# cbg-ethz/LongSom

Hardware: AMD Instinct MI355X
Metric: genomic sites/s pileup+call, 10M-read BAM x 5k barcodes, 1/2/4/8 MI355X (higher is better)
Workload: dtype u32

## Files before the change

### longsom_amd/csrc/pileup.hip

```cpp
#include "lsg_ctx.h"
#include <hipcub/hipcub.hpp>
#include <cstdio>
#include <cstdlib>
#include <cstring>

namespace lsg {

#define LSG_AS3 __attribute__((address_space(3)))
__device__ __forceinline__ uint32_t lds_addr(const void* p) { return (uint32_t)(uintptr_t)(LSG_AS3 const void*)p; }
constexpr int ARENA = 256;

enum { SC_COLS = 8, SC_OVERFLOW = 9, SC_READS = 10, SC_SEGS = 11, SC_EVENTS = 12, SC_ROWS_DEEP = 15,
       SC_ROWS = 16, SC_ROWS_SRC = 28, SC_NENT = 38, SC_QWALK = 48,
       SC_ROWALLOC = 160, SC_ROWALLOC_STRIDE = 16, SC_COUNT = SC_ROWALLOC + SC_ROWALLOC_STRIDE * LSG_MAX_CELLTYPES };

struct CountArgs {
    int64_t n_reads;
    const int32_t* read_tid; const uint16_t* read_flag; const uint8_t* read_mapq; const int32_t* read_cb;
    const int64_t* contig_len; const uint8_t* const* ref_ptr;
    const uint8_t* celltype_of;
    int32_t n_contigs, n_cb, n_ct;
    uint32_t tile_lo, tile_hi;
    int32_t min_bq, min_mq, min_dp, min_cc, ignore_orphans;
    uint32_t flag_exclude;
// ... 15 lines not shown
    unsigned long long n_ok = 0;
    for (int64_t r = (int64_t)blockIdx.x * blockDim.x + threadIdx.x; r < a.n_reads; r += (int64_t)gridDim.x * blockDim.x) {
        const uint32_t flag = a.read_flag[r];
        const int32_t cb = a.read_cb[r], tid = a.read_tid[r];
        bool pass = (flag & a.flag_exclude) == 0 && (int)a.read_mapq[r] >= a.min_mq;
        if (pass && a.ignore_orphans && (flag & 0x1) && !(flag & 0x2)) pass = false;
        if (pass && a.read_drop && a.read_drop[r] == 1) pass = false;
        if (a.adm) {
            const unsigned long long m = __ballot(pass);
            if ((threadIdx.x & 63) == 0) a.adm[r >> 6] = m;
        }
        bool ok = pass && cb >= 0 && cb < a.n_cb && tid >= 0 && tid < a.n_contigs;
        if (ok && a.celltype_of[cb] >= (uint32_t)a.n_ct) ok = false;
        n_ok += ok;
    }
    __shared__ unsigned long long s_ok;
    if (threadIdx.x == 0) s_ok = 0;
    __syncthreads();
    for (int o = 32; o > 0; o >>= 1) n_ok += __shfl_down(n_ok, o);
    if ((threadIdx.x & 63) == 0 && n_ok) atomicAdd(&s_ok, n_ok);
    __syncthreads();
    if (threadIdx.x == 0 && s_ok) atomicAdd(&a.scalars[SC_READS], s_ok);
}

__device__ __forceinline__ void lds_fence() {
    __builtin_amdgcn_fence(__ATOMIC_ACQ_REL, "workgroup");
    __builtin_amdgcn_wave_barrier();
}
__device__ __forceinline__ uint32_t rl(uint32_t v, int l) { return (uint32_t)__builtin_amdgcn_readlane((int)v, l); }
__device__ __forceinline__ uint32_t bq_threshold(const CountArgs& a) {
    const int q = a.min_bq < 0 ? 0 : (a.min_bq > 256 ? 256 : a.min_bq);
    return 0x800u + (uint32_t)q;
}

struct WaveBook {
    uint32_t arena_next[LSG_MAX_CELLTYPES], arena_end[LSG_MAX_CELLTYPES], rows_true[LSG_MAX_CELLTYPES];
    uint32_t cols, rows_deep, rows_src, src;
    unsigned long long nev;
};
__device__ __forceinline__ void book_init(WaveBook& b, int lane) {
    if (lane < LSG_MAX_CELLTYPES) { b.arena_next[lane] = 0; b.arena_end[lane] = 0; b.rows_true[lane] = 0; }
    if (lane == 0) { b.cols = 0; b.rows_deep = 0; b.rows_src = 0; b.src = 0; }
}
__device__ __forceinline__ void book_flush(const CountArgs& a, WaveBook& b, int lane) {
    lds_fence();
    if (lane < a.n_ct && b.rows_true[lane]) atomicAdd(&a.scalars[SC_ROWS + lane], (unsigned long long)b.rows_true[lane]);
    if (lane == 0 && b.cols) atomicAdd(&a.scalars[SC_COLS], (unsigned long long)b.cols);
    if (lane == 0 && b.rows_deep) atomicAdd(&a.scalars[SC_ROWS_DEEP], (unsigned long long)b.rows_deep);
    if (lane == 0 && b.rows_src) atomicAdd(&a.scalars[SC_ROWS_SRC + b.src], (unsigned long long)b.rows_src);
}

template <class CNT, bool NARROW = false>
__device__ __forceinline__ void emit_unit(const CountArgs& a, const CNT& acc, uint32_t w, int ct, int tid, int32_t tstart, int lane,
                                          WaveBook* bk, bool deep, int ref_prefetched = -1, int arena_slot = -1) {
    const int as = arena_slot < 0 ? ct : arena_slot;
    uint32_t dp = 0;
#pragma unroll
    for (int s = 0; s < 8; ++s) dp += acc.BC(s);
    const uint32_t nc = dp - acc.NCDUP();
    int64_t pos = (int64_t)tstart + lane;
    bool valid = pos >= 1 && pos < a.contig_len[tid];
    uint8_t refb = 'N';
    if (ref_prefetched >= 0) refb = (uint8_t)ref_prefetched;
    else if (valid) refb = a.ref_ptr[tid][pos];
    unsigned long long colm = __ballot(valid && dp > 0);
    bool emit = valid && dp > 0 && (int)dp >= a.min_dp && (int)nc >= a.min_cc && refb != 'N';
    unsigned long long em = __ballot(emit);
    const uint32_t k = (uint32_t)__popcll(em);
    uint32_t base = 0;
    if (lane == 0) {
        if (bk) {
            bk->cols += (uint32_t)__popcll(colm);
            if (k) {
                uint32_t nx = bk->arena_next[as];
                if (nx + k > bk->arena_end[as]) {
                    nx = (uint32_t)atomicAdd(&a.scalars[SC_ROWALLOC + SC_ROWALLOC_STRIDE * ct], (unsigned long long)a.arena);
                    bk->arena_end[as] = nx + a.arena;
                }
                base = nx; bk->arena_next[as] = nx + k; bk->rows_true[ct] += k;
                if (deep) bk->rows_deep += k;
                bk->rows_src += k;
            }
        } else {
            if (colm) atomicAdd(&a.scalars[SC_COLS], (unsigned long long)__popcll(colm));
            if (k) {
                base = (uint32_t)atomicAdd(&a.scalars[SC_ROWALLOC + SC_ROWALLOC_STRIDE * ct], (unsigned long long)k);
                atomicAdd(&a.scalars[SC_ROWS + ct], (unsigned long long)k);
                if (deep) atomicAdd(&a.scalars[SC_ROWS_DEEP], (unsigned long long)k);
                atomicAdd(&a.scalars[SC_ROWS_SRC + 3], (unsigned long long)k);
            }
        }
        a.ne_mask[w] = em;
        a.ne_rowbase[w] = base | (NARROW ? ROW_NARROW : 0u);
    }
    base = rl(base, 0);
    if (!em) return;
    if ((uint64_t)base + k > a.row_cap) {
        if (lane == 0) atomicExch(&a.scalars[SC_OVERFLOW], 1ull);
        return;
    }
    if (!emit) return;
    const uint32_t row = base + (uint32_t)__popcll(em & ((1ull << lane) - 1ull));
    const uint32_t b0 = base >> 6;
    const uint32_t off16 = (((row >> 6) - b0) * (uint32_t)ROW_BLOCK_WORDS + (row & 63u) * 4u) * 4u;
    const uint64_t first = (uint64_t)(uintptr_t)a.rows[ct] + (uint64_t)b0 * (ROW_BLOCK_WORDS * 4ull);
    const uint64_t p0 = ((uint64_t)rl((uint32_t)(first >> 32), 0) << 32) | rl((uint32_t)first, 0);
    const __amdgpu_buffer_rsrc_t rs = __builtin_amdgcn_make_buffer_rsrc(reinterpret_cast<void*>((uintptr_t)p0), 0, (int)(2 * ROW_BLOCK_WORDS * 4), 0x00020000);
    typedef uint32_t u32x4 __attribute__((ext_vector_type(4)));
    auto plane = [&](int p) -> uint32_t {
        if (p == 0) return dp;
        if (p == 1) return nc;
        if (p < 10) return acc.BC(p - 2) - acc.DUP(p - 2);
        if (p < 18) return acc.BC(p - 10);
        if (p < 26) return acc.BQ(p - 18);
        if (p < 34) return acc.BCF(p - 26);
        return 0u;
    };
    if (NARROW) {
        typedef uint32_t u32x2 __attribute__((ext_vector_type(2)));
        const uint32_t off8 = ((row >> 6) - b0) * (uint32_t)ROW_BLOCK_WORDS * 4u + (row & 63u) * 8u;
#pragma unroll
        for (int q = 0; q < ROW_QUADS; ++q) {
            u32x2 v; v.x = plane(4 * q) | (plane(4 * q + 1) << 16); v.y = plane(4 * q + 2) | (plane(4 * q + 3) << 16);
            __builtin_amdgcn_raw_buffer_store_b64(v, rs, (int)off8, q * 512, 0);
            asm volatile("s_nop 3");
            __builtin_amdgcn_sched_barrier(0);
        }
        return;
    }
#pragma unroll
    for (int q = 0; q < ROW_QUADS; ++q) {
        u32x4 v; v.x = plane(4 * q); v.y = plane(4 * q + 1); v.z = plane(4 * q + 2); v.w = plane(4 * q + 3);
        __builtin_amdgcn_raw_buffer_store_b128(v, rs, (int)off16, q * 1024, 0);
        asm volatile("s_nop 3");
        __builtin_amdgcn_sched_barrier(0);
    }
}

struct Acc {
    uint32_t bc[8], bq[8], bcf[8], dup[8], ncdup;
    __device__ __forceinline__ void init() {
#pragma unroll
        for (int s = 0; s < 8; ++s) bc[s] = bq[s] = bcf[s] = dup[s] = 0;
        ncdup = 0;
    }
    __device__ __forceinline__ uint32_t BC(int s) const { return bc[s]; }
    __device__ __forceinline__ uint32_t BQ(int s) const { return bq[s]; }
    __device__ __forceinline__ uint32_t BCF(int s) const { return bcf[s]; }
    __device__ __forceinline__ uint32_t DUP(int s) const { return dup[s]; }
    __device__ __forceinline__ uint32_t NCDUP() const { return ncdup; }
};

constexpr int FIN_THREADS = 512;
__global__ __launch_bounds__(FIN_THREADS) void k_finalize_multi(CountArgs a) {
    __shared__ uint32_t sacc[NCTR][64];
    __shared__ WaveBook book;
    const int t = threadIdx.x, lane = t & 63, wv = t >> 6;
    if (wv == 0) { book_init(book, lane); if (lane == 0) book.src = 3; }
    for (uint32_t k = blockIdx.x; k < a.n_multi; k += gridDim.x) {
        const uint32_t w = a.multi_list[k];
        const uint32_t nslot = a.ne_nslot[w];
        { const uint32_t tile = a.ne_units[w] / (uint32_t)a.n_ct; if (tile < a.tile_lo || tile >= a.tile_hi) continue; }
        __syncthreads();
        for (int i = t; i < NCTR * 64; i += FIN_THREADS) (&sacc[0][0])[i] = 0;
        __syncthreads();
        Acc tot; tot.init();
        for (uint32_t j = wv; j < nslot; j += FIN_THREADS / 64) {
            const uint32_t* src = a.macc + (uint64_t)(a.ne_acc[w] + j) * (NCTR * 64);
            tot.ncdup += src[lane];
#pragma unroll
            for (int sy = 0; sy < 8; ++sy) {
                tot.dup[sy] += src[(1 + sy) * 64 + lane]; tot.bc[sy] += src[(9 + sy) * 64 + lane];
                tot.bq[sy] += src[(17 + sy) * 64 + lane]; tot.bcf[sy] += src[(25 + sy) * 64 + lane];
            }
        }
        if ((uint32_t)wv < nslot) {
            atomicAdd(&sacc[0][lane], tot.ncdup);
#pragma unroll
            for (int sy = 0; sy < 8; ++sy) {
                atomicAdd(&sacc[1 + sy][lane], tot.dup[sy]); atomicAdd(&sacc[9 + sy][lane], tot.bc[sy]);
                atomicAdd(&sacc[17 + sy][lane], tot.bq[sy]); atomicAdd(&sacc[25 + sy][lane], tot.bcf[sy]);
            }
        }
        __syncthreads();
        if (wv == 0) {
            tot.ncdup = sacc[0][lane];
#pragma unroll
            for (int sy = 0; sy < 8; ++sy) {
                tot.dup[sy] = sacc[1 + sy][lane]; tot.bc[sy] = sacc[9 + sy][lane];
                tot.bq[sy] = sacc[17 + sy][lane]; tot.bcf[sy] = sacc[25 + sy][lane];
            }
            const int2 geom = a.ne_geom[w];
            emit_unit(a, tot, w, (int)((uint32_t)geom.y >> 24), geom.y & 0xffffff, geom.x, lane, &book, true);
        }
    }
    if (wv == 0) book_flush(a, book, lane);
}

static int read_scalars(lsg_ctx* c, unsigned long long* sc) {
    LSG_HIP(hipMemcpyAsync(c->h_pin, c->d_scalars.p, SC_COUNT * 8, hipMemcpyDeviceToHost, c->stream));
    LSG_HIP(hipStreamSynchronize(c->stream));
    memcpy(sc, c->h_pin, SC_COUNT * 8);
    return 0;
}

static void fill_args(lsg_ctx* c, const lsg_count_params* p, CountArgs& a) {
    a.n_reads = c->rd.n_reads;
    a.read_tid = c->rd.read_tid; a.read_flag = c->rd.read_flag; a.read_mapq = c->rd.read_mapq; a.read_cb = c->rd.read_cb;
    a.contig_len = c->d_contig_len.as<int64_t>();
    a.ref_ptr = c->d_ref_ptrs.as<const uint8_t*>(); a.celltype_of = c->d_celltype_of.as<uint8_t>();
    a.n_contigs = c->n_contigs; a.n_cb = c->n_cb; a.n_ct = c->n_ct;
    a.tile_lo = c->tile_lo; a.tile_hi = c->tile_hi;
    a.min_bq = p->min_bq; a.min_mq = p->min_mq; a.min_dp = p->min_dp; a.min_cc = p->min_cc;
    a.ignore_orphans = p->ignore_orphans; a.flag_exclude = p->flag_exclude;
    a.read_drop = c->has_drops ? c->d_read_drop.as<uint8_t>() : nullptr;
    a.drop_pairs = c->has_drops && c->n_drop_pairs ? c->d_drop_pairs.as<unsigned long long>() : nullptr; a.n_drop_pairs = c->n_drop_pairs;
    a.tile_base = c->d_tile_base.as<uint32_t>(); a.window = c->st_window;
    const bool all_in = !c->has_drops && p->min_mq <= c->st_min_mq && (p->flag_exclude & ~c->st_flag_exclude) == 0 && (!p->ignore_orphans || c->st_ignore_orphans);
    a.adm = all_in ? nullptr : c->d_read_adm.as<unsigned long long>();
    a.ne_units = c->d_ne_units.as<uint32_t>(); a.ne_nslot = c->ws[WS_NE_NSLOT].as<uint32_t>();
    a.ne_acc = c->ws[WS_NE_ACC].as<uint32_t>(); a.ne_geom = c->ws[WS_NE_GEOM].as<int2>();
    a.ne_mask = c->d_ne_mask.as<uint64_t>(); a.ne_rowbase = c->d_ne_rowbase.as<uint32_t>();
    a.multi_list = c->ws[WS_MULTI_LIST].as<uint32_t>(); a.macc = c->ws[WS_MACC].as<uint32_t>();
    a.n_ne = c->n_ne; a.n_multi = c->n_multi;
    a.scalars = c->d_scalars.as<unsigned long long>();
    for (int i = 0; i < LSG_MAX_CELLTYPES; ++i) a.rows[i] = c->d_rows[i].as<uint32_t>();
    a.row_cap = c->row_cap; a.arena = c->arena;
}

static int tune_int(const char* name, int dflt) {
    const char* v = getenv(name);
    if (!v || !*v) return dflt;
    const int x = atoi(v);
    return x > 0 && x <= 64 ? x : dflt;
}

#define SCAN_U32(in, out, n)                                                                              \
    do {                                                                                                  \
        size_t tb_ = 0;                                                                                   \
        LSG_HIP(hipcub::DeviceScan::ExclusiveSum(nullptr, tb_, (in), (out), (int)(n), st));              \
        if (c->d_cub_tmp.reserve(tb_ + 256)) return -1;                                                   \
        tb_ = c->d_cub_tmp.cap;                                                                           \
        LSG_HIP(hipcub::DeviceScan::ExclusiveSum(c->d_cub_tmp.p, tb_, (in), (out), (int)(n), st));       \
    } while (0)

#ifndef LSG_TM_ASM
#define LSG_TM_ASM true
#endif
constexpr int IX_STAT_SLOTS = 256;
// ... 275 lines not shown
        for (int k = 0; k < TM_GROUP; ++k) {
            if ((uint32_t)g * TM_GROUP + k >= nblk) break;
#pragma unroll
            for (int u = 0; u < 8; ++u) {
                const uint32_t m = rl(M, k * 8 + u);
                if (u & 1) tm_add<true>(st, m, E[k][u >> 1], thr, pkl0, one);
                else tm_add<false>(st, m, E[k][u >> 1], thr, pkl0, one);
            }
        }
    };
    issue(0, EA, MA);
    int g = 0;
    while (true) {
        if (g + 1 < ng) issue(g + 1, EB, MB);
        consume(g, EA, MA);
        if (++g >= ng) break;
        if (g + 1 < ng) issue(g + 1, EA, MA);
        consume(g, EB, MB);
        if (++g >= ng) break;
    }
    st.nc += st.mask & 0x10001u; st.mask = 0;
}

struct JobRec {
    uint32_t e0, e1, w0, slab, nj, tcnt, tile, emid, base, off; int32_t tstart; int tid;
    __device__ __forceinline__ void load(uint32_t jw) {
        e0 = rl(jw, 0); e1 = rl(jw, 1); w0 = rl(jw, 2); slab = rl(jw, 3); nj = rl(jw, 4); tcnt = rl(jw, 5); tile = rl(jw, 6); emid = rl(jw, 7); base = rl(jw, 8); off = rl(jw, 9);
        tstart = (int32_t)rl(jw, 10); tid = (int)rl(jw, 11);
    }
};
template <int PLANE_WORDS, int NC_WORDS>
__device__ __forceinline__ void tm_zero_planes(uint32_t* pl, uint32_t* nc_sh) {
#pragma unroll
    for (int i = 0; i < PLANE_WORDS / (4 * TMW_WAVES * 64); ++i) reinterpret_cast<uint4*>(pl)[i * (TMW_WAVES * 64) + threadIdx.x] = make_uint4(0u, 0u, 0u, 0u);
#pragma unroll
    for (int i = 0; i < NC_WORDS / (TMW_WAVES * 64); ++i) nc_sh[i * (TMW_WAVES * 64) + threadIdx.x] = 0;
}
template <class CNT>
__device__ __forceinline__ void tm_finish(const CountArgs& a, const uint32_t* pc, uint32_t nc, uint32_t unit, uint32_t slab, uint32_t nj, uint32_t tcnt, int ct, int tid, int32_t tstart,
                                          int lane, WaveBook* book, int refb, int arena_slot) {
    CNT tot{pc, lane, 0u};
    uint32_t dp = 0;
#pragma unroll
    for (int k = 0; k < 8; ++k) dp += tot.BC(k);
    tot.ncdup = dp - nc;
    if (nj == 1) {
        if (tcnt <= ROW_NARROW_MAX) emit_unit<CNT, true>(a, tot, unit, ct, tid, tstart, lane, book, false, refb, arena_slot);
        else emit_unit<CNT, false>(a, tot, unit, ct, tid, tstart, lane, book, false, refb, arena_slot + 1);
    } else {
        uint32_t* dst = a.macc + (uint64_t)slab * (NCTR * 64);
        dst[lane] = tot.NCDUP();
#pragma unroll
        for (int k = 0; k < 8; ++k) {
            dst[(1 + k) * 64 + lane] = tot.DUP(k); dst[(9 + k) * 64 + lane] = tot.BC(k);
            dst[(17 + k) * 64 + lane] = tot.BQ(k); dst[(25 + k) * 64 + lane] = tot.BCF(k);
        }
    }
}
__device__ __forceinline__ void books_flush(const CountArgs& a, const WaveBook (&books)[TMW_WAVES], int lane) {
    if (threadIdx.x < 64) {
        uint32_t rt = 0, cols = 0, rsrc = 0;
        for (int w = 0; w < TMW_WAVES; ++w) {
            const WaveBook& b = books[w];
            if (lane < a.n_ct) rt += b.rows_true[lane];
            cols += b.cols; rsrc += b.rows_src;
        }
        if (lane < a.n_ct && rt) atomicAdd(&a.scalars[SC_ROWS + lane], (unsigned long long)rt);
        if (lane == 0) {
            if (cols) atomicAdd(&a.scalars[SC_COLS], (unsigned long long)cols);
            if (rsrc) atomicAdd(&a.scalars[SC_ROWS_SRC + 1], (unsigned long long)rsrc);
        }
    }
}
struct TgStat { uint32_t ev, sg, ne; };
__device__ __forceinline__ void stat_add(unsigned long long* stat_slots, uint32_t who, unsigned long long ev, unsigned long long sg, unsigned long long ne, int lane) {
    if (lane == 0 && ne) {
        unsigned long long* slot = stat_slots + (size_t)(who % IX_STAT_SLOTS) * 8;
        atomicAdd(&slot[0], ev); atomicAdd(&slot[1], sg); atomicAdd(&slot[2], ne);
    }
}
__device__ __forceinline__ void stat_flush(unsigned long long* stat_slots, const TgStat& stat, int lane, int wv) {
    unsigned long long ev = stat.ev, sg = stat.sg, ne = stat.ne;
    for (int o = 32; o > 0; o >>= 1) { ev += __shfl_down(ev, o); sg += __shfl_down(sg, o); ne += __shfl_down(ne, o); }
    stat_add(stat_slots, blockIdx.x * TMW_WAVES + wv, ev, sg, ne, lane);
}

__global__ __launch_bounds__(TMW_WAVES * 64) __attribute__((amdgpu_waves_per_eu(8))) void k_tm_walk(CountArgs a, TmArgs tm) {
    __shared__ __attribute__((aligned(8192))) uint32_t planes[2][2][8 * 64];
    __shared__ uint32_t nc_sh[2][64];
    __shared__ WaveBook books[TMW_WAVES];
    __shared__ uint32_t s_ck;
    const int lane = threadIdx.x & 63, wv = __builtin_amdgcn_readfirstlane((int)(threadIdx.x >> 6));
    uint32_t* pl = &planes[0][0][0];
    WaveBook& book = books[wv];
    book_init(book, lane);
    if (lane == 0) book.src = 1;
    const uint32_t thr = bq_threshold(a), pkl0 = lds_addr(pl + lane);
    uint32_t one = 1u;
    asm volatile("" : "+v"(one));
    for (bool first = true;; first = false) {
        __syncthreads();
        if (threadIdx.x == 0) s_ck = first ? blockIdx.x : (uint32_t)atomicAdd(&a.scalars[SC_QWALK], 1ull) + gridDim.x;
        __syncthreads();
        const uint32_t ck = rl(s_ck, 0);
        if (ck >= tm.nchunks) break;
        const uint32_t jx_end = rl(tm.chunk_start[ck + 1], 0);
        for (uint32_t jx = rl(tm.chunk_start[ck], 0); jx < jx_end; ++jx) {
            uint32_t jw = 0;
// ... 861 lines not shown
        if (cls < 2)
            for (int h = 0; h < H; ++h) { const uint32_t q = (uint32_t)(64 * h + lane) - first; if (q < nev) e.ev[h] = tg.events[src + q]; }
        return e;
    }
};
static_assert(TM_JOB_TGT <= TM_JOB_LIMIT, "a one-job tile's job fits the packed planes: the wide walk writes slabs only");
template <class SRC>
__global__ __launch_bounds__(64) void k_tm_walk_wide(CountArgs a, TmArgs tm, SRC src, const uint32_t* n_wide) {
    constexpr int H = SRC::H;
    __shared__ uint32_t pl[H][2][4][8 * 64];
    const int lane = threadIdx.x;
    if (n_wide && rl(*n_wide, 0) == 0u) return;
    const uint32_t thr = bq_threshold(a);
    unsigned long long s_ev = 0, s_sg = 0, s_ne = 0;
    for (uint32_t jx = blockIdx.x; jx < tm.njobs; jx += gridDim.x) {
        const TmJob jb = tm.jobs[jx];
        bool in_t[H], any = false;
        for (int h = 0; h < H; ++h) { const uint32_t t = (uint32_t)H * jb.tile + h; in_t[h] = t >= a.tile_lo && t < a.tile_hi; any |= in_t[h]; }
        if (!(jb.nj & TMJ_WIDE) || !any) continue;
        const uint32_t nj = jb.nj & ~TMJ_WIDE;
        lds_fence();
        for (int i = lane; i < H * 2 * 4 * 8 * 64; i += 64) (&pl[0][0][0][0])[i] = 0;
        lds_fence();
        uint32_t nc[H][2], mask[H], run_ct = 0;
        for (int h = 0; h < H; ++h) { nc[h][0] = nc[h][1] = 0; mask[h] = 0; }
        for (uint32_t p = jb.e0; p < jb.e1 && p - jb.base < jb.cnt; ++p) {
            const WideEntry e = src.entry(a, tm, jb, p, lane);
            if (e.rs) for (int h = 0; h < H; ++h) { nc[h][run_ct] += mask[h] ? 1u : 0u; mask[h] = 0; }
            if (e.cls >= 2) continue;
            s_ev += e.nev; s_sg += e.segfirst ? 1u : 0u; ++s_ne;
            run_ct = e.cls;
            for (int h = 0; h < H; ++h) {
                const uint32_t ev = e.ev[h];
                if ((ev & 0x8ffu) >= thr) {
                    const uint32_t sym = (ev >> 8) & 7u;
                    uint32_t* w = &pl[h][run_ct][0][sym * 64 + lane];
                    w[0] += ev & 0xffu; w[512] += e.fwd ? 1u : 0u; w[1024] += 1u; w[1536] += (mask[h] >> sym) & 1u;
                    mask[h] |= 1u << sym;
                }
            }
        }
        for (int h = 0; h < H; ++h) nc[h][run_ct] += mask[h] ? 1u : 0u;
        lds_fence();
        for (int h = 0; h < H; ++h) {
            if (!in_t[h]) continue;
            for (int v = 0; v < 2; ++v) {
                const int ct = tm.ct_base + v;
                if (ct >= a.n_ct) break;
                const uint32_t* pc = &pl[h][v][0][0];
                uint32_t dp = 0;
#pragma unroll
                for (int k = 0; k < 8; ++k) dp += pc[1024 + k * 64 + lane];
                uint32_t* dst = a.macc + (uint64_t)(jb.slab + ((uint32_t)h * (uint32_t)a.n_ct + (uint32_t)ct) * nj) * (NCTR * 64);
                dst[lane] = dp - nc[h][v];
#pragma unroll
                for (int k = 0; k < 8; ++k) {
                    dst[(1 + k) * 64 + lane] = pc[1536 + k * 64 + lane]; dst[(9 + k) * 64 + lane] = pc[1024 + k * 64 + lane];
                    dst[(17 + k) * 64 + lane] = pc[k * 64 + lane]; dst[(25 + k) * 64 + lane] = pc[512 + k * 64 + lane];
                }
            }
        }
    }
    if (unsigned long long* slots = src.stat_slots()) stat_add(slots, blockIdx.x, s_ev, s_sg, s_ne, lane);
}

struct CountLaunch { CountArgs a; TmArgs tm; unsigned grid_walk, grid_fin; int n_pass; };
struct PrepOp { void* dst; const void* src; uint64_t words; };
struct PrepArgs { PrepOp op[10]; int n; };
__global__ __launch_bounds__(256) void k_prep_ops(PrepArgs a) {
    const uint64_t g = (uint64_t)blockIdx.x * blockDim.x + threadIdx.x, gs = (uint64_t)gridDim.x * blockDim.x;
    for (int k = 0; k < a.n; ++k) {
        uint32_t* d = reinterpret_cast<uint32_t*>(a.op[k].dst);
        const uint32_t* sp = reinterpret_cast<const uint32_t*>(a.op[k].src);
        const uint64_t nq = a.op[k].words / 4;
        for (uint64_t i = g; i < nq; i += gs) reinterpret_cast<uint4*>(d)[i] = sp ? reinterpret_cast<const uint4*>(sp)[i] : make_uint4(0u, 0u, 0u, 0u);
        for (uint64_t i = nq * 4 + g; i < a.op[k].words; i += gs) d[i] = sp ? sp[i] : 0u;
    }
}
static int count_prepare(lsg_ctx* c, const lsg_count_params* p, CountLaunch& L) {
    hipStream_t st = c->stream;
    const uint32_t n_ne = c->tm_n_ne;
    if (c->d_scalars.reserve(SC_COUNT * 8) || c->d_ne_units.reserve(((size_t)n_ne + 2) * 4) ||
        c->d_ne_mask.reserve(((size_t)n_ne + 2) * 8) || c->d_ne_rowbase.reserve(((size_t)n_ne + 2) * 4) || c->ws[WS_NE_NSLOT].reserve(((size_t)n_ne + 2) * 4) ||
        c->ws[WS_NE_ACC].reserve(((size_t)n_ne + 2) * 4) || c->ws[WS_NE_GEOM].reserve(((size_t)n_ne + 2) * 8) || c->ws[WS_MULTI_LIST].reserve(((size_t)c->tm_n_multi + 2) * 4) ||
        c->ws[WS_MACC].reserve(((size_t)c->tm_n_slabs + 1) * NCTR * 64 * 4) || c->d_ix_stat.reserve(IX_STAT_SLOTS * 64) ||
        c->d_read_adm.reserve(((size_t)c->rd.n_reads / 64 + 2) * 8))
        return -1;
    L.grid_walk = (unsigned)(c->n_cus * tune_int("LSG_GRID_TM", 16));
    L.grid_fin = (unsigned)(c->n_cus * 8);
    L.n_pass = (c->n_ct + 1) / 2;
    {
        uint64_t want_rows = (uint64_t)n_ne / (uint64_t)c->n_ct * TILE_W;
        if (p->min_dp > 0) {
            const uint64_t by_depth = (uint64_t)c->rd.n_events / (uint64_t)p->min_dp + 64;
            if (by_depth < want_rows) want_rows = by_depth;
        }
        const uint64_t emitters = (uint64_t)L.grid_walk * TMW_WAVES * 2 + L.grid_fin + (uint64_t)c->n_cus * 4 + (c->wsh ? (uint64_t)c->n_cus * 16 * TMW_WAVES * 4 : 0u);
        uint64_t arena = want_rows / (emitters * 8) / ARENA * ARENA;
        c->arena = (uint32_t)(arena < (uint64_t)ARENA ? (uint64_t)ARENA : (arena > 8ull * ARENA ? 8ull * ARENA : arena));
        want_rows += emitters * c->arena + 64;
        want_rows = (want_rows + 63) / 64 * 64 + 64;
        if (want_rows > c->row_cap) c->row_cap = want_rows;
        for (int i = 0; i < c->n_ct; ++i)
            if (c->d_rows[i].reserve((size_t)c->row_cap * ROW_STORED_WORDS * 4)) return -1;
    }
    c->n_ne = n_ne; c->n_multi = c->tm_n_multi;
    L.a = CountArgs{};
    fill_args(c, p, L.a);
    TmArgs& tm = L.tm;
    tm = TmArgs{};
    tm.store = c->tm[TM_STORE].as<uint4>(); tm.s0 = c->tm[TM_S0].as<uint32_t>(); tm.b = c->tm[TM_B].as<uint8_t>(); tm.rd = c->tm[TM_RD].as<uint32_t>();
    tm.meta = c->tm[TM_META].as<uint32_t>(); tm.blk_tile = c->tm[TM_BLK_TILE].as<uint32_t>(); tm.jobs = c->tm[TM_JOBS].as<TmJob>(); tm.np = c->tm_np; tm.nblk = c->tm_nblk;
    tm.njobs = c->tm_njobs; tm.nchunks = c->tm_nchunks; tm.chunk_start = c->tm[TM_CHUNKS].as<uint32_t>(); tm.ext = c->tm[TM_EXT].as<uint16_t>();
    LSG_HIP(hipEventRecord(c->ev[0], st));
    {
        PrepArgs pa{}; int k = 0;
        auto op = [&](void* dst, const void* src, size_t bytes) { if (bytes) { pa.op[k].dst = dst; pa.op[k].src = src; pa.op[k].words = (bytes + 3) / 4; ++k; } };
        op(c->d_scalars.p, nullptr, SC_COUNT * 8);
        op(c->d_ix_stat.p, nullptr, IX_STAT_SLOTS * 64);
        if (n_ne) {
            op(c->d_ne_units.p, c->tm[TM_NE_UNITS].p, (size_t)n_ne * 4);
            op(c->ws[WS_NE_GEOM].p, c->tm[TM_NE_GEOM].p, (size_t)n_ne * 8);
            op(c->ws[WS_NE_NSLOT].p, c->tm[TM_NE_NSLOT].p, ((size_t)n_ne + 1) * 4);
            op(c->ws[WS_NE_ACC].p, c->tm[TM_NE_ACC].p, ((size_t)n_ne + 1) * 4);
            if (c->tm_n_multi) op(c->ws[WS_MULTI_LIST].p, c->tm[TM_MULTI].p, (size_t)c->tm_n_multi * 4);
            op(c->d_ne_mask.p, nullptr, ((size_t)n_ne + 1) * 8);
            op(c->d_ne_rowbase.p, nullptr, ((size_t)n_ne + 1) * 4);
        }
        pa.n = k;
        hipLaunchKernelGGL(k_prep_ops, dim3((unsigned)(c->n_cus * 4)), dim3(256), 0, st, pa);
    }
    const int64_t R = c->rd.n_reads;
    if (R > 0) { unsigned g = (unsigned)((R + 255) / 256); if (g > (unsigned)(c->n_cus * 8)) g = (unsigned)(c->n_cus * 8); hipLaunchKernelGGL(k_read_stats, dim3(g), dim3(256), 0, st, L.a); }
    return 0;
}
static int count_passes(lsg_ctx* c, CountLaunch& L, int first_pass, bool wide_of_pass0) {
    hipStream_t st = c->stream;
    const unsigned grid_wide = c->tm_n_wide ? (c->tm_n_wide < (unsigned)(c->n_cus * 4) ? c->tm_n_wide : (unsigned)(c->n_cus * 4)) : 0u;
    for (int pass = wide_of_pass0 ? 0 : first_pass; pass < L.n_pass && c->tm_nblk; ++pass) {
        const bool wide_only = pass < first_pass;
        if (wide_only && !grid_wide) continue;
        L.tm.ct_base = 2 * pass;
        if (pass) LSG_HIP(hipMemsetAsync(L.a.scalars + SC_QWALK, 0, 8, st));
        if (L.a.drop_pairs) hipLaunchKernelGGL(k_tm_resolve<true>, dim3((c->tm_nblk + 255) / 256), dim3(256), 0, st, L.a, L.tm, wide_only ? (unsigned long long*)nullptr : c->d_ix_stat.as<unsigned long long>());
        else hipLaunchKernelGGL(k_tm_resolve<false>, dim3((c->tm_nblk + 255) / 256), dim3(256), 0, st, L.a, L.tm, wide_only ? (unsigned long long*)nullptr : c->d_ix_stat.as<unsigned long long>());
        if (pass == 0) { LSG_HIP(hipEventRecord(c->ev[1], st)); LSG_HIP(hipEventRecord(c->ev[3], st)); }
        if (c->tm_njobs && !wide_only) hipLaunchKernelGGL(k_tm_walk, dim3(L.grid_walk), dim3(TMW_WAVES * 64), 0, st, L.a, L.tm);
        if (pass == 0) LSG_HIP(hipEventRecord(c->ev[4], st));
        if (grid_wide) hipLaunchKernelGGL(k_tm_walk_wide<WideFromStore>, dim3(grid_wide), dim3(64), 0, st, L.a, L.tm, WideFromStore{0}, (const uint32_t*)nullptr);
    }
    return 0;
}
static int count_finish(lsg_ctx* c, const lsg_count_params* p, CountLaunch& L) {
    hipStream_t st = c->stream;
    if (c->tm_nblk) hipLaunchKernelGGL(k_resolve_stats, dim3(1), dim3(256), 0, st, L.a, c->d_ix_stat.as<unsigned long long>());
    if (c->tm_n_multi) hipLaunchKernelGGL(k_finalize_multi, dim3(c->tm_n_multi < L.grid_fin ? c->tm_n_multi : L.grid_fin), dim3(FIN_THREADS), 0, st, L.a);
    LSG_HIP(hipEventRecord(c->ev[5], st));
    LSG_HIP(hipGetLastError());
    unsigned long long sc[SC_COUNT];
    if (read_scalars(c, sc)) return -1;
    if (sc[SC_OVERFLOW]) { set_error("lsg_pileup_count: row buffer overflow (cap %llu)", (unsigned long long)c->row_cap); return -3; }
    for (int i = 0; i < LSG_MAX_CELLTYPES; ++i) c->n_rows[i] = (int64_t)sc[SC_ROWS + i];
    c->n_columns = (int64_t)sc[SC_COLS];
    c->stats.n_reads_admitted = (int64_t)sc[SC_READS];
    c->stats.n_segs_admitted = (int64_t)sc[SC_SEGS];
    c->stats.n_events_admitted = (int64_t)sc[SC_EVENTS];
    c->stats.n_units = c->n_ne;
    c->stats.n_deep_units = c->tm_n_multi;
    c->stats.n_entries = (int64_t)sc[SC_NENT];
    float ms = 0;
    LSG_HIP(hipEventElapsedTime(&ms, c->ev[0], c->ev[1])); c->stats.ms_bin = ms;
    LSG_HIP(hipEventElapsedTime(&ms, c->ev[1], c->ev[5])); c->stats.ms_deep = ms;
    LSG_HIP(hipEventElapsedTime(&ms, c->ev[3], c->ev[4])); c->stats.ms_walk = ms;
    c->stats.ms_wave = 0;
    LSG_HIP(hipEventElapsedTime(&ms, c->ev[0], c->ev[5])); c->stats.ms_total = ms;
    for (int i = 0; i < 4; ++i) { c->stats.rows_by_kernel[i] = (int64_t)sc[SC_ROWS_SRC + i]; c->stats.events_by_kernel[i] = 0; }
    c->stats.events_by_kernel[1] = (int64_t)sc[SC_EVENTS];
    c->stats.n_events_wave = 0; c->stats.n_events_deep = (int64_t)sc[SC_EVENTS];
    c->stats.n_rows_deep = (int64_t)sc[SC_ROWS_DEEP];
    c->stats.n_rows_wave = -c->stats.n_rows_deep;
    for (int i = 0; i < LSG_MAX_CELLTYPES; ++i) c->stats.n_rows_wave += c->n_rows[i];
    c->last_params = *p;
    c->counted = true;
    c->called = false;
    ++c->count_serial;
    return 0;
}

int run_gather_count(lsg_ctx* c, const lsg_count_params* p, const GatherCountSrc& src, bool direct) {
    hipStream_t st = c->stream;
    c->has_drops = false; c->n_depth_dropped = 0;
    CountLaunch L;
    if (int rc = count_prepare(c, p, L)) return rc;
    TgArgs tg{};
    tg.events = src.events; tg.n_events = src.n_events; tg.key = src.key; tg.rdv = src.rdv; tg.cb_bits = src.cb_bits;
    tg.src_mask = (1ull << ((src.rdv ? 52 : 50) - src.cb_bits)) - 1ull; tg.src_shift = src.src_shift;
    if (!src.rdv && (!direct || L.a.adm)) return 1;
    tg.tile_off = c->d_tile_off.as<uint32_t>(); tg.blk_off = c->tm[TM_BLK_OFF].as<uint32_t>();
    tg.s0 = c->tm[TM_S0].as<uint32_t>(); tg.b8 = c->tm[TM_B].as<uint8_t>(); tg.rd = c->tm[TM_RD].as<uint32_t>();
    tg.store = c->tm[TM_STORE].as<uint4>(); tg.ext = c->tm[TM_EXT].as<uint16_t>();
    tg.nchunks = c->d_plan_misc + 1; tg.stat_slots = c->d_ix_stat.as<unsigned long long>();
    L.tm.ct_base = 0;
    const bool dbg = getenv("LSG_DEBUG_SYNC") != nullptr;
    auto stage = [&](const char* what) { if (dbg) { const hipError_t e = hipStreamSynchronize(st); fprintf(stderr, "[lsg] fused load: %s: %s\n", what, hipGetErrorString(e)); fflush(stderr); } };
    stage("count prepared");
    LSG_HIP(hipEventRecord(c->ev[1], st)); LSG_HIP(hipEventRecord(c->ev[3], st));
    enum { GATHER, TILES, WINDOWS } form = !direct ? GATHER : (src.wsh ? WINDOWS : TILES);
    const char* what = "k_tm_gather_count";
    if (direct) {
// ... 134 lines not shown
```

### longsom_amd/csrc/store.hip

```cpp
#include "lsg_ctx.h"
#include <hipcub/hipcub.hpp>
#include <chrono>
#include <cstdio>
#include <cstdlib>
#include <utility>

namespace lsg {

constexpr uint32_t KEY_INVALID = 0xFFFFFFFFu;

constexpr uint32_t RV_WHI = 1u << 29, RV_SEGFIRST = 1u << 30, RV_FWD = 1u << 31, RV_READ = RV_WHI - 1u;
__host__ __device__ __forceinline__ uint64_t sort_key(uint32_t cb, uint32_t first, uint32_t nev1, uint64_t src, int cb_bits, int wsh = 0) {
    return (uint64_t)cb | ((uint64_t)(first | (nev1 << (6 + wsh))) << cb_bits) | (src << (cb_bits + 12 + 2 * wsh));
}

struct BuildArgs {
    int64_t n_reads, n_segs, n_events;
    const int32_t* read_tid; const uint16_t* read_flag; const uint8_t* read_mapq; const int32_t* read_cb;
    const uint32_t* seg_read; const int32_t* seg_start; const int32_t* seg_len; const int64_t* seg_ev_off;
    const uint32_t* tile_base; const int64_t* contig_len;
    int32_t n_contigs; uint32_t n_tiles;
    uint2* seg_info;
    uint32_t* tile_cap;
    uint32_t* cursor;
// ... 1092 lines not shown
    return 0;
}

static int plan_jobs(lsg_ctx* c, bool finish, const uint64_t* skey, int cb_bits) {
    hipStream_t st = c->stream;
    const RunSrc rs{c->tm[TM_S0].as<uint32_t>(), skey, skey ? (1u << cb_bits) - 1u : 0u};
    const uint32_t T = c->n_tiles >> c->wsh;
    DevBuf &per_tile = c->bt[BT_PER_TILE], &offs = c->bt[BT_OFFS];
    uint32_t* nj = per_tile.as<uint32_t>() + (T + 2);
    uint32_t* ne_off = offs.as<uint32_t>(); uint32_t* job_off = ne_off + (T + 2); uint32_t* slab_off = job_off + (T + 2); uint32_t* multi_off = slab_off + (T + 2);
    uint32_t* d_misc = multi_off + (T + 2);
    const uint32_t* tot = c->plan1_tot;
    const uint32_t njobs = tot[1], n_mt = tot[3];
    hipLaunchKernelGGL(k_tm_jobs, dim3((T + 255) / 256), dim3(256), 0, st, c->d_tile_base.as<uint32_t>(), c->n_contigs, c->n_ct, c->wsh, rs, c->d_tile_off.as<uint32_t>(),
                       c->d_tile_cap.as<uint32_t>(), c->tm[TM_BLK_OFF].as<uint32_t>(), ne_off, nj, job_off, slab_off, multi_off, T,
                       c->tm[TM_JOBS].as<TmJob>(), c->tm[TM_NE_UNITS].as<uint32_t>(), c->tm[TM_NE_GEOM].as<int2>(), c->tm[TM_NE_NSLOT].as<uint32_t>(),
                       c->tm[TM_NE_ACC].as<uint32_t>(), c->tm[TM_MULTI].as<uint32_t>(), d_misc);
    if (n_mt) hipLaunchKernelGGL(k_tm_jobs_multi, dim3(n_mt >> c->wsh), dim3(64), 0, st, c->n_ct, c->wsh, rs, c->d_tile_off.as<uint32_t>(), c->d_tile_cap.as<uint32_t>(), c->tm[TM_BLK_OFF].as<uint32_t>(),
                                 ne_off, nj, job_off, slab_off, c->tm[TM_MULTI].as<uint32_t>(), c->tm[TM_NE_UNITS].as<uint32_t>(), c->tm[TM_NE_GEOM].as<int2>(), n_mt >> c->wsh, c->tm[TM_JOBS].as<TmJob>(), d_misc);
    {
        DevBuf& pex = c->bt[BT_PEX];
        const uint64_t total_work = c->tm_np + (uint64_t)njobs * TM_JOB_W0;
        const uint64_t cw = total_work / ((uint64_t)c->n_cus * 14 * 6);
        const uint32_t chunk_work = (uint32_t)(cw < 256 ? 256 : (cw > TM_CHUNK_WORK ? TM_CHUNK_WORK : cw));
        if (pex.reserve(((size_t)njobs + 2) * 4) || c->tm[TM_CHUNKS].reserve(((size_t)(total_work / chunk_work) + 4) * 4)) return -1;
        hipcub::CountingInputIterator<uint32_t> iota(0);
        TmJobWork wf{c->tm[TM_JOBS].as<TmJob>()};
        hipcub::TransformInputIterator<uint32_t, TmJobWork, hipcub::CountingInputIterator<uint32_t>> it(iota, wf);
        SCAN_U32(it, pex.as<uint32_t>(), njobs);
        hipLaunchKernelGGL(k_tm_chunks, dim3((njobs + 255) / 256), dim3(256), 0, st, pex.as<uint32_t>(), njobs, chunk_work, c->tm[TM_CHUNKS].as<uint32_t>(), d_misc + 1);
    }
    LSG_HIP(hipMemcpyAsync(c->plan_misc, d_misc, 8, hipMemcpyDeviceToHost, st));
    c->d_plan_misc = d_misc;
    LSG_HIP(hipGetLastError());
    if (finish) LSG_HIP(hipStreamSynchronize(st));
    return 0;
}

static void plan_finish_tiles(lsg_ctx* c) {
    const uint32_t* tot = c->plan1_tot;
    c->tm_njobs = tot[1];
    c->tm_n_ne = (uint32_t)((size_t)tot[0] * (size_t)c->n_ct); c->tm_n_multi = (uint32_t)((size_t)tot[3] * (size_t)c->n_ct); c->tm_n_slabs = tot[2];
}
static void plan_finish(lsg_ctx* c) {
    plan_finish_tiles(c);
    c->tm_nchunks = c->plan_misc[1]; c->tm_n_wide = c->plan_misc[0];
    c->plan_n_ct = c->n_ct;
    if (getenv("LSG_TIMING")) {
        std::vector<TmJob> jobs(c->tm_njobs);
        uint32_t longest = 0;
        if (c->tm_njobs && hipMemcpy(jobs.data(), c->tm[TM_JOBS].p, (size_t)c->tm_njobs * sizeof(TmJob), hipMemcpyDeviceToHost) != hipSuccess) { (void)hipGetLastError(); return; }
        for (const TmJob& jb : jobs) if (!(jb.nj & TMJ_WIDE) && jb.e1 - jb.e0 > longest) longest = jb.e1 - jb.e0;
        fprintf(stderr, "[lsg] plan: %u jobs, %u multi-job tiles, %u wide, longest packed job %u entries\n", c->tm_njobs, c->plan1_tot[3], c->tm_n_wide, longest);
    }
}

int ensure_plan(lsg_ctx* c) {
    if (!c->tm_valid) { set_error("lsg_pileup_count: no reads loaded"); return -2; }
    if (c->plan_n_ct == c->n_ct) return 0;
    c->plan_n_ct = 0;
    c->tm_njobs = c->tm_nchunks = c->tm_n_ne = c->tm_n_multi = c->tm_n_slabs = c->tm_n_wide = 0;
    if (c->tm_nblk == 0) { c->plan_n_ct = c->n_ct; return 0; }
    if (c->plan1_n_ct != c->n_ct) { if (int rc = plan_tiles(c, c->stream)) return rc; }
    if (int rc = plan_jobs(c, true)) return rc;
    plan_finish(c);
    return 0;
}

}
```

Before: 3.626 billion.

## Pack multi-job slabs into 17 planes and finalize small units per wave

Narrow job slabs now store quality sum and forward count in one word and count and duplicates in another. This cuts the per-slab planes read in the finalize kernel from 33 to 17, and wide slabs are tagged with a high bit in plane 0. The finalize kernel now handles units with few slabs one per wave, with software double-buffered slab loads and prefetched unit metadata. Units above a tunable slab threshold keep the block-wide LDS reduction path, and the finalize grid is reduced. Packing relies on static bounds on job size, and a timing-only slab histogram is added to the plan printout.

```diff
diff --git a/longsom_amd/csrc/pileup.hip b/longsom_amd/csrc/pileup.hip
--- a/longsom_amd/csrc/pileup.hip
+++ b/longsom_amd/csrc/pileup.hip
@@ -91,14 +91,14 @@
 
 template <class CNT, bool NARROW = false>
 __device__ __forceinline__ void emit_unit(const CountArgs& a, const CNT& acc, uint32_t w, int ct, int tid, int32_t tstart, int lane,
-                                          WaveBook* bk, bool deep, int ref_prefetched = -1, int arena_slot = -1) {
+                                          WaveBook* bk, bool deep, int ref_prefetched = -1, int arena_slot = -1, int64_t clen_prefetched = -1) {
     const int as = arena_slot < 0 ? ct : arena_slot;
     uint32_t dp = 0;
 #pragma unroll
     for (int s = 0; s < 8; ++s) dp += acc.BC(s);
     const uint32_t nc = dp - acc.NCDUP();
     int64_t pos = (int64_t)tstart + lane;
-    bool valid = pos >= 1 && pos < a.contig_len[tid];
+    bool valid = pos >= 1 && pos < (clen_prefetched >= 0 ? clen_prefetched : a.contig_len[tid]);
     uint8_t refb = 'N';
     if (ref_prefetched >= 0) refb = (uint8_t)ref_prefetched;
     else if (valid) refb = a.ref_ptr[tid][pos];
@@ -190,50 +190,170 @@
     __device__ __forceinline__ uint32_t NCDUP() const { return ncdup; }
 };
 
-constexpr int FIN_THREADS = 512;
-__global__ __launch_bounds__(FIN_THREADS) void k_finalize_multi(CountArgs a) {
+constexpr int SLAB_PLANES = 17;
+constexpr uint32_t SLAB_WIDE = 1u << 31;
+static_assert(TM_JOB_LIMIT * 255 < (1 << 20), "packed slab, plane 1 + 2k: a job's quality sum of 8-bit qualities fits bits 0..19");
+static_assert(TM_JOB_LIMIT < (1 << 12), "packed slab, plane 1 + 2k: a job's forward count fits bits 20..31");
+static_assert(TM_JOB_LIMIT < (1 << 16) && TM_JOB_LIMIT - 1 < (1 << 16), "packed slab, plane 2 + 2k: a job's count fits bits 0..15, its duplicates bits 16..31");
+static_assert((uint32_t)TM_JOB_LIMIT < SLAB_WIDE, "packed slab, plane 0: NCDUP of a job leaves bit 31 clear");
+static_assert(SLAB_PLANES == 1 + 2 * 8 && SLAB_PLANES <= NCTR, "a packed slab lies in the first planes of the plan's slab");
+
+__device__ __forceinline__ void slab_load(uint32_t (&r)[SLAB_PLANES], const uint32_t* macc, uint32_t slab, int lane) {
+    const uint32_t* src = macc + (uint64_t)slab * (NCTR * 64) + lane;
+#pragma unroll
+    for (int p = 0; p < SLAB_PLANES; ++p) r[p] = src[p * 64];
+}
+__device__ __forceinline__ void slab_add(Acc& tot, const uint32_t (&r)[SLAB_PLANES], const uint32_t* macc, uint32_t slab, int lane) {
+    if (!(rl(r[0], 0) & SLAB_WIDE)) {
+        tot.ncdup += r[0];
+#pragma unroll
+        for (int k = 0; k < 8; ++k) {
+            tot.bq[k] += r[1 + 2 * k] & 0xfffffu; tot.bcf[k] += r[1 + 2 * k] >> 20;
+            tot.bc[k] += r[2 + 2 * k] & 0xffffu; tot.dup[k] += r[2 + 2 * k] >> 16;
+        }
+    } else {
+        const uint32_t* src = macc + (uint64_t)slab * (NCTR * 64) + lane;
+        tot.ncdup += r[0] & ~SLAB_WIDE;
+#pragma unroll
+        for (int k = 0; k < 8; ++k) {
+            tot.dup[k] += r[1 + k]; tot.bc[k] += r[9 + k];
+            tot.bq[k] += src[(17 + k) * 64]; tot.bcf[k] += src[(25 + k) * 64];
+        }
+        asm volatile("" : "+v"(tot.ncdup), "+v"(tot.bc[0]), "+v"(tot.bc[1]), "+v"(tot.bc[2]), "+v"(tot.bc[3]), "+v"(tot.bc[4]), "+v"(tot.bc[5]), "+v"(tot.bc[6]), "+v"(tot.bc[7]),
+                          "+v"(tot.dup[0]), "+v"(tot.dup[1]), "+v"(tot.dup[2]), "+v"(tot.dup[3]), "+v"(tot.dup[4]), "+v"(tot.dup[5]), "+v"(tot.dup[6]), "+v"(tot.dup[7]));
+        asm volatile("" : "+v"(tot.bq[0]), "+v"(tot.bq[1]), "+v"(tot.bq[2]), "+v"(tot.bq[3]), "+v"(tot.bq[4]), "+v"(tot.bq[5]), "+v"(tot.bq[6]), "+v"(tot.bq[7]),
+                          "+v"(tot.bcf[0]), "+v"(tot.bcf[1]), "+v"(tot.bcf[2]), "+v"(tot.bcf[3]), "+v"(tot.bcf[4]), "+v"(tot.bcf[5]), "+v"(tot.bcf[6]), "+v"(tot.bcf[7]));
+    }
+}
+
+template <class T> __device__ __forceinline__ T sload(const T* p, uint64_t i) { return reinterpret_cast<const __attribute__((address_space(4))) T*>((uintptr_t)p)[i]; }
+struct FinUnit { uint32_t w, nslot, acc; int32_t tstart; uint32_t tidct; int64_t clen; int refb; };
+__device__ __forceinline__ FinUnit fin_unit(const CountArgs& a, uint64_t& k, uint64_t stride, uint32_t fin_s, int lane) {
+    FinUnit u{0u, 0u, 0u, 0, 0u, 0, 'N'};
+    for (; k < a.n_multi; k += stride) {
+        const uint32_t w = sload(a.multi_list, k);
+        const uint32_t nslot = sload(a.ne_nslot, w), tile = sload(a.ne_units, w) / (uint32_t)a.n_ct;
+        if (tile < a.tile_lo || tile >= a.tile_hi || nslot > fin_s || nslot == 0) continue;
+        const uint64_t geom = sload(reinterpret_cast<const uint64_t*>(a.ne_geom), w);
+        u.w = w; u.nslot = nslot; u.acc = sload(a.ne_acc, w); u.tstart = (int32_t)(uint32_t)geom; u.tidct = (uint32_t)(geom >> 32);
+        const int tid = (int)(u.tidct & 0xffffffu);
+        const int64_t pos = (int64_t)u.tstart + lane;
+        u.clen = sload(a.contig_len, tid);
+        if (pos >= 1 && pos < u.clen) u.refb = sload(a.ref_ptr, tid)[pos];
+        k += stride;
+        break;
+    }
+    return u;
+}
+constexpr int FIN_THREADS = 512, FIN_WAVES = FIN_THREADS / 64;
+constexpr int FIN_S = 8;
+__device__ __forceinline__ void fin_books_flush(const CountArgs& a, const WaveBook (&books)[FIN_WAVES], int lane) {
+    if (threadIdx.x < 64) {
+        uint32_t rt = 0, cols = 0, rsrc = 0, deep = 0;
+        for (int w = 0; w < FIN_WAVES; ++w) {
+            const WaveBook& b = books[w];
+            if (lane < a.n_ct) rt += b.rows_true[lane];
+            cols += b.cols; rsrc += b.rows_src; deep += b.rows_deep;
+        }
+        if (lane < a.n_ct && rt) atomicAdd(&a.scalars[SC_ROWS + lane], (unsigned long long)rt);
+        if (lane == 0) {
+            if (cols) atomicAdd(&a.scalars[SC_COLS], (unsigned long long)cols);
+            if (deep) atomicAdd(&a.scalars[SC_ROWS_DEEP], (unsigned long long)deep);
+            if (rsrc) atomicAdd(&a.scalars[SC_ROWS_SRC + 3], (unsigned long long)rsrc);
+        }
+    }
+}
+
+__global__ __launch_bounds__(FIN_THREADS) __attribute__((amdgpu_waves_per_eu(4, 4))) void k_finalize_multi(CountArgs a, uint32_t fin_s) {
     __shared__ uint32_t sacc[NCTR][64];
-    __shared__ WaveBook book;
-    const int t = threadIdx.x, lane = t & 63, wv = t >> 6;
-    if (wv == 0) { book_init(book, lane); if (lane == 0) book.src = 3; }
-    for (uint32_t k = blockIdx.x; k < a.n_multi; k += gridDim.x) {
-        const uint32_t w = a.multi_list[k];
-        const uint32_t nslot = a.ne_nslot[w];
-        { const uint32_t tile = a.ne_units[w] / (uint32_t)a.n_ct; if (tile < a.tile_lo || tile >= a.tile_hi) continue; }
+    __shared__ WaveBook books[FIN_WAVES];
+    __shared__ unsigned long long s_big[FIN_WAVES];
+    const int t = threadIdx.x, lane = t & 63, wv = __builtin_amdgcn_readfirstlane(t >> 6);
+    WaveBook& book = books[wv];
+    book_init(book, lane);
+    for (uint64_t k0 = blockIdx.x; k0 < a.n_multi; k0 += (uint64_t)FIN_THREADS * gridDim.x) {
+        const uint64_t kt = k0 + (uint64_t)t * gridDim.x;
+        bool big = false;
+        if (kt < a.n_multi) {
+            const uint32_t w = a.multi_list[kt], tile = a.ne_units[w] / (uint32_t)a.n_ct;
+            big = a.ne_nslot[w] > fin_s && tile >= a.tile_lo && tile < a.tile_hi;
+        }
+        const unsigned long long bm = __ballot(big);
         __syncthreads();
-        for (int i = t; i < NCTR * 64; i += FIN_THREADS) (&sacc[0][0])[i] = 0;
+        if (lane == 0) s_big[wv] = bm;
         __syncthreads();
-        Acc tot; tot.init();
-        for (uint32_t j = wv; j < nslot; j += FIN_THREADS / 64) {
-            const uint32_t* src = a.macc + (uint64_t)(a.ne_acc[w] + j) * (NCTR * 64);
-            tot.ncdup += src[lane];
-#pragma unroll
-            for (int sy = 0; sy < 8; ++sy) {
-                tot.dup[sy] += src[(1 + sy) * 64 + lane]; tot.bc[sy] += src[(9 + sy) * 64 + lane];
-                tot.bq[sy] += src[(17 + sy) * 64 + lane]; tot.bcf[sy] += src[(25 + sy) * 64 + lane];
+        for (int v = 0; v < FIN_WAVES; ++v) {
+            unsigned long long m = s_big[v];
+            m = ((unsigned long long)rl((uint32_t)(m >> 32), 0) << 32) | rl((uint32_t)m, 0);
+            while (m) {
+                const int bit = __builtin_ctzll(m);
+                m &= m - 1;
+                const uint32_t w = rl(a.multi_list[k0 + (uint64_t)(v * 64 + bit) * gridDim.x], 0);
+                const uint32_t nslot = rl(a.ne_nslot[w], 0), acc0 = rl(a.ne_acc[w], 0);
+                __syncthreads();
+                for (int i = t; i < NCTR * 64; i += FIN_THREADS) (&sacc[0][0])[i] = 0;
+                __syncthreads();
+                Acc tot; tot.init();
+                for (uint32_t j = (uint32_t)wv; j < nslot; j += FIN_WAVES) {
+                    uint32_t r[SLAB_PLANES];
+                    slab_load(r, a.macc, acc0 + j, lane);
+                    slab_add(tot, r, a.macc, acc0 + j, lane);
+                }
+                if ((uint32_t)wv < nslot) {
+                    atomicAdd(&sacc[0][lane], tot.ncdup);
+#pragma unroll
+                    for (int sy = 0; sy < 8; ++sy) {
+                        atomicAdd(&sacc[1 + sy][lane], tot.dup[sy]); atomicAdd(&sacc[9 + sy][lane], tot.bc[sy]);
+                        atomicAdd(&sacc[17 + sy][lane], tot.bq[sy]); atomicAdd(&sacc[25 + sy][lane], tot.bcf[sy]);
+                    }
+                }
+                __syncthreads();
+                if (wv == 0) {
+                    tot.ncdup = sacc[0][lane];
+#pragma unroll
+                    for (int sy = 0; sy < 8; ++sy) {
+                        tot.dup[sy] = sacc[1 + sy][lane]; tot.bc[sy] = sacc[9 + sy][lane];
+                        tot.bq[sy] = sacc[17 + sy][lane]; tot.bcf[sy] = sacc[25 + sy][lane];
+                    }
+                    const int2 geom = a.ne_geom[w];
+                    emit_unit(a, tot, w, (int)((uint32_t)geom.y >> 24), geom.y & 0xffffff, geom.x, lane, &book, true);
+                }
             }
         }
-        if ((uint32_t)wv < nslot) {
-            atomicAdd(&sacc[0][lane], tot.ncdup);
-#pragma unroll
-            for (int sy = 0; sy < 8; ++sy) {
-                atomicAdd(&sacc[1 + sy][lane], tot.dup[sy]); atomicAdd(&sacc[9 + sy][lane], tot.bc[sy]);
-                atomicAdd(&sacc[17 + sy][lane], tot.bq[sy]); atomicAdd(&sacc[25 + sy][lane], tot.bcf[sy]);
+    }
+    {
+        const uint64_t stride = (uint64_t)FIN_WAVES * gridDim.x;
+        uint64_t nk = (uint64_t)blockIdx.x * FIN_WAVES + (uint64_t)wv;
+        FinUnit cu = fin_unit(a, nk, stride, fin_s, lane);
+        while (cu.nslot) {
+            uint32_t ra[SLAB_PLANES], rb[SLAB_PLANES];
+            slab_load(ra, a.macc, cu.acc, lane);
+            FinUnit nu = fin_unit(a, nk, stride, fin_s, lane);
+            const uint32_t ahead = nu.acc;
+            Acc tot; tot.init();
+#define LSG_FIN_WAIT(r) asm volatile("" : "+v"(r[0]), "+v"(r[1]), "+v"(r[2]), "+v"(r[3]), "+v"(r[4]), "+v"(r[5]), "+v"(r[6]), "+v"(r[7]), "+v"(r[8]), "+v"(r[9]), \
+                                      "+v"(r[10]), "+v"(r[11]), "+v"(r[12]), "+v"(r[13]), "+v"(r[14]), "+v"(r[15]), "+v"(r[16]) : : "memory")
+            for (uint32_t j = 0;; j += 2) {
+                const bool more1 = j + 1 < cu.nslot;
+                slab_load(rb, a.macc, more1 ? cu.acc + j + 1 : ahead, lane);
+                LSG_FIN_WAIT(ra);
+                asm volatile("" : "+v"(nu.refb));
+                slab_add(tot, ra, a.macc, cu.acc + j, lane);
+                if (!more1) break;
+                const bool more2 = j + 2 < cu.nslot;
+                slab_load(ra, a.macc, more2 ? cu.acc + j + 2 : ahead, lane);
+                LSG_FIN_WAIT(rb);
+                slab_add(tot, rb, a.macc, cu.acc + j + 1, lane);
+                if (!more2) break;
             }
-        }
-        __syncthreads();
-        if (wv == 0) {
-            tot.ncdup = sacc[0][lane];
-#pragma unroll
-            for (int sy = 0; sy < 8; ++sy) {
-                tot.dup[sy] = sacc[1 + sy][lane]; tot.bc[sy] = sacc[9 + sy][lane];
-                tot.bq[sy] = sacc[17 + sy][lane]; tot.bcf[sy] = sacc[25 + sy][lane];
-            }
-            const int2 geom = a.ne_geom[w];
-            emit_unit(a, tot, w, (int)((uint32_t)geom.y >> 24), geom.y & 0xffffff, geom.x, lane, &book, true);
-        }
-    }
-    if (wv == 0) book_flush(a, book, lane);
+#undef LSG_FIN_WAIT
+            emit_unit(a, tot, cu.w, (int)(cu.tidct >> 24), (int)(cu.tidct & 0xffffffu), cu.tstart, lane, &book, true, cu.refb, -1, cu.clen);
+            cu = nu;
+        }
+    }
+    lds_fence();
+    __syncthreads();
+    fin_books_flush(a, books, lane);
 }
 
 static int read_scalars(lsg_ctx* c, unsigned long long* sc) {
@@ -615,8 +735,7 @@
         dst[lane] = tot.NCDUP();
 #pragma unroll
         for (int k = 0; k < 8; ++k) {
-            dst[(1 + k) * 64 + lane] = tot.DUP(k); dst[(9 + k) * 64 + lane] = tot.BC(k);
-            dst[(17 + k) * 64 + lane] = tot.BQ(k); dst[(25 + k) * 64 + lane] = tot.BCF(k);
+            dst[(1 + 2 * k) * 64 + lane] = tot.BQ(k) | (tot.BCF(k) << 20); dst[(2 + 2 * k) * 64 + lane] = tot.BC(k) | (tot.DUP(k) << 16);
         }
     }
 }
@@ -1584,7 +1703,7 @@
 #pragma unroll
                 for (int k = 0; k < 8; ++k) dp += pc[1024 + k * 64 + lane];
                 uint32_t* dst = a.macc + (uint64_t)(jb.slab + ((uint32_t)h * (uint32_t)a.n_ct + (uint32_t)ct) * nj) * (NCTR * 64);
-                dst[lane] = dp - nc[h][v];
+                dst[lane] = (dp - nc[h][v]) | SLAB_WIDE;
 #pragma unroll
                 for (int k = 0; k < 8; ++k) {
                     dst[(1 + k) * 64 + lane] = pc[1536 + k * 64 + lane]; dst[(9 + k) * 64 + lane] = pc[1024 + k * 64 + lane];
@@ -1596,7 +1715,7 @@
     if (unsigned long long* slots = src.stat_slots()) stat_add(slots, blockIdx.x, s_ev, s_sg, s_ne, lane);
 }
 
-struct CountLaunch { CountArgs a; TmArgs tm; unsigned grid_walk, grid_fin; int n_pass; };
+struct CountLaunch { CountArgs a; TmArgs tm; unsigned grid_walk, grid_fin; uint32_t fin_s; int n_pass; };
 struct PrepOp { void* dst; const void* src; uint64_t words; };
 struct PrepArgs { PrepOp op[10]; int n; };
 __global__ __launch_bounds__(256) void k_prep_ops(PrepArgs a) {
@@ -1619,7 +1738,8 @@
         c->d_read_adm.reserve(((size_t)c->rd.n_reads / 64 + 2) * 8))
         return -1;
     L.grid_walk = (unsigned)(c->n_cus * tune_int("LSG_GRID_TM", 16));
-    L.grid_fin = (unsigned)(c->n_cus * 8);
+    L.grid_fin = (unsigned)(c->n_cus * 2);
+    L.fin_s = (uint32_t)tune_int("LSG_FIN_S", FIN_S);
     L.n_pass = (c->n_ct + 1) / 2;
     {
         uint64_t want_rows = (uint64_t)n_ne / (uint64_t)c->n_ct * TILE_W;
@@ -1627,7 +1747,7 @@
             const uint64_t by_depth = (uint64_t)c->rd.n_events / (uint64_t)p->min_dp + 64;
             if (by_depth < want_rows) want_rows = by_depth;
         }
-        const uint64_t emitters = (uint64_t)L.grid_walk * TMW_WAVES * 2 + L.grid_fin + (uint64_t)c->n_cus * 4 + (c->wsh ? (uint64_t)c->n_cus * 16 * TMW_WAVES * 4 : 0u);
+        const uint64_t emitters = (uint64_t)L.grid_walk * TMW_WAVES * 2 + (uint64_t)L.grid_fin * FIN_WAVES + (uint64_t)c->n_cus * 4 + (c->wsh ? (uint64_t)c->n_cus * 16 * TMW_WAVES * 4 : 0u);
         uint64_t arena = want_rows / (emitters * 8) / ARENA * ARENA;
         c->arena = (uint32_t)(arena < (uint64_t)ARENA ? (uint64_t)ARENA : (arena > 8ull * ARENA ? 8ull * ARENA : arena));
         want_rows += emitters * c->arena + 64;
@@ -1686,7 +1806,10 @@
 static int count_finish(lsg_ctx* c, const lsg_count_params* p, CountLaunch& L) {
     hipStream_t st = c->stream;
     if (c->tm_nblk) hipLaunchKernelGGL(k_resolve_stats, dim3(1), dim3(256), 0, st, L.a, c->d_ix_stat.as<unsigned long long>());
-    if (c->tm_n_multi) hipLaunchKernelGGL(k_finalize_multi, dim3(c->tm_n_multi < L.grid_fin ? c->tm_n_multi : L.grid_fin), dim3(FIN_THREADS), 0, st, L.a);
+    if (c->tm_n_multi) {
+        const unsigned need = (c->tm_n_multi + FIN_WAVES - 1) / FIN_WAVES;
+        hipLaunchKernelGGL(k_finalize_multi, dim3(need < L.grid_fin ? need : L.grid_fin), dim3(FIN_THREADS), 0, st, L.a, L.fin_s);
+    }
     LSG_HIP(hipEventRecord(c->ev[5], st));
     LSG_HIP(hipGetLastError());
     unsigned long long sc[SC_COUNT];
diff --git a/longsom_amd/csrc/store.hip b/longsom_amd/csrc/store.hip
--- a/longsom_amd/csrc/store.hip
+++ b/longsom_amd/csrc/store.hip
@@ -1168,6 +1168,16 @@
         if (c->tm_njobs && hipMemcpy(jobs.data(), c->tm[TM_JOBS].p, (size_t)c->tm_njobs * sizeof(TmJob), hipMemcpyDeviceToHost) != hipSuccess) { (void)hipGetLastError(); return; }
         for (const TmJob& jb : jobs) if (!(jb.nj & TMJ_WIDE) && jb.e1 - jb.e0 > longest) longest = jb.e1 - jb.e0;
         fprintf(stderr, "[lsg] plan: %u jobs, %u multi-job tiles, %u wide, longest packed job %u entries\n", c->tm_njobs, c->plan1_tot[3], c->tm_n_wide, longest);
+        std::vector<uint32_t> nslot(c->tm_n_ne);
+        if (c->tm_n_ne && hipMemcpy(nslot.data(), c->tm[TM_NE_NSLOT].p, (size_t)c->tm_n_ne * 4, hipMemcpyDeviceToHost) != hipSuccess) { (void)hipGetLastError(); return; }
+        unsigned long long units = 0, slabs = 0, by[6] = {0, 0, 0, 0, 0, 0}, sl[6] = {0, 0, 0, 0, 0, 0};
+        for (const uint32_t n : nslot) {
+            if (n < 2) continue;
+            const int b = n <= 2 ? 1 : n <= 4 ? 2 : n <= 8 ? 3 : n <= 16 ? 4 : 5;
+            ++units; slabs += n; ++by[b]; sl[b] += n;
+        }
+        fprintf(stderr, "[lsg] slabs: %llu multi-job units, %llu slabs; units (their slabs) of 1: %llu (%llu), 2: %llu (%llu), 3-4: %llu (%llu), 5-8: %llu (%llu), 9-16: %llu (%llu), more: %llu (%llu)\n",
+                units, slabs, by[0], sl[0], by[1], sl[1], by[2], sl[2], by[3], sl[3], by[4], sl[4], by[5], sl[5]);
     }
 }
 
```

New measurement: 3.556 billion. -1.9%, worse.
